# qmoututu11/Image_Restoration_and_Enhancement

Measured on AMD Instinct MI355X. Metric: restored images/sec @512x512, 50 DDIM steps; PSNR/SSIM vs reference, higher is better.
Workload: dtype bf16; 1 GPU; BASELINE configs[1] denoise 512x512, batch 8/GPU, 50 DDIM steps x strength 0.5 = 25 UNet evals, CFG 5.0 (UNet batch 16); task=denoise, global_batch=8, resolution=512, compute=UNet + CLIP bf16, VAE fp16 (fp32 accumulation), parallelism=dp1, weights_bcast=none, outputs_finite=True

## Files before the change

image_restoration_and_enhancement_amd/csrc/gemm_plan.cpp:

```cpp
#include "gemm_plan.h"

#include <algorithm>
#include <cmath>

namespace irx {

bool g_large_tiles = true;
int g_large_mask = 3;
int g_large_dense = 63;
int g_small_splitk = 1;
int g_gemm_sk = 1;
int g_gemm_deep = 0;
bool g_gemm_small = false;
int g_gemm_small_kmax = 1280;
int g_gemm_force = 0;
bool g_tile_256x320 = true;
bool g_splitk_inkernel = true;
int g_gemm_nmajor = 1;
int g_gemm_group = 1;
int g_gemm_pp = 2;
int g_gemm_pp2 = 1;
int g_gemm_pp_chain = 1;
int g_conv1x1_dense = 1;
int g_conv_halo = 1;
int g_halo_split = 1;
int g_halo_pipe = 1;
int g_halo_strip = 1;
int g_halo_up2 = 1;
int g_halo_mi = 1;
int g_halo_group = 1;
int g_gn_fuse = 0;
int g_gn_parts = 1;
int g_gn_red_parts = 1;
int g_gn_fold = 1;
int g_ln_fold = 1;
int g_ln_parts = 1;

namespace {

constexpr int kCUs = 256;
constexpr long kPairMinTiles = 2L * kCUs;

struct Choice {
  int BM = 0, BN = 0, splits = 1, per = 0;
  bool small = false;
  bool pair = false;
};

int step_k() { return g_gemm_deep == 1 ? 32 : 64; }

long canon_rows(const GemmArgs& a) {
  const long rows = (long)a.M * a.batch;
  return a.imgs > 0 ? rows / a.imgs * kCanonImages : rows;
}
int canon_batch(const GemmArgs& a) { return (a.imgs > 0 && a.batch > 1) ? kCanonImages : a.batch; }

bool reduce_in_kernel(int splits, long tiles) { return g_splitk_inkernel && splits == 2 && tiles <= kSplitCounters; }

Choice choose(const GemmArgs& a) {
  Choice best;
  const int nk = std::max(1, a.K / step_k());
  if (g_gemm_small && g_gemm_deep == 0 && a.K <= g_gemm_small_kmax) {
    const int bn = (!a.geglu && a.N % 160 == 0) ? 160 : (a.N % 128 == 0 ? 128 : 0);
    if (bn) {
      best.BM = 128; best.BN = bn; best.small = true; best.splits = 1; best.per = nk;
      return best;
    }
  }
  if (g_gemm_force > 0 && g_gemm_deep == 0) {
    const int BM = g_gemm_force / 100000, BN = (g_gemm_force / 100) % 1000, sp = g_gemm_force % 100;
    const bool ok = (BM == 256 || BM == 128 || (BM == 64 && BN == 320 && sp == 1 && !a.gn_part)) &&
                    (BN == 320 || BN == 256 || BN == 128) && a.N % BN == 0 &&
                    sp >= 1 && (sp == 1 || !((a.out_f32 && canon_batch(a) > 1) || a.geglu)) && (!a.geglu || BN % 128 == 0);
    if (ok) {
      best.BM = BM; best.BN = BN; best.splits = sp; best.per = (nk + sp - 1) / sp;
      if ((long)(sp - 1) * best.per < nk) return best;
    }
    best = Choice();
  }
  double best_score = -1.0;
  const int cands[7][2] = {{256, 320}, {256, 256}, {128, 320}, {256, 128}, {128, 256}, {128, 128}, {256, 160}};
  for (auto& c : cands) {
    const int BM = c[0], BN = c[1];
    if (BN == 160 && g_gemm_deep != 2) continue;
    if (BN == 320 && BM == 256 && (g_gemm_deep != 0 || !g_tile_256x320)) continue;
    if (a.N % BN != 0) continue;
    if (a.geglu && BN % 128 != 0) continue;
    const long tiles = (canon_rows(a) + BM - 1) / BM * (a.N / BN);
    const double eff = BM == 256 ? (BN >= 256 ? 1.0 : BN == 160 ? 0.9 : 0.65)
                                 : (BN == 320 ? 0.97 : BN == 256 ? 0.75 : 0.78);
    const int resident = (BM == 128 && BN == 128 && g_gemm_deep == 0) ? 2 : 1;
    const long cap = (long)kCUs * resident;
    for (int splits = 1; splits <= 8; splits *= 2) {
      if (splits > 1 && ((a.out_f32 && canon_batch(a) > 1) || a.geglu)) break;
      const int per = (nk + splits - 1) / splits;
      if (per * step_k() < 512 && splits > 1) break;
      if ((long)(splits - 1) * per >= nk) break;
      const long blocks = tiles * splits;
      const double util = (double)blocks / ((double)((blocks + cap - 1) / cap) * cap);
      const double cost_split = splits > 1 ? (1.0 + 0.35 * std::log2((double)splits)) * (per < 16 ? 1.6 : 1.0) : 1.0;
      const double score = util * eff / cost_split;
      if (score > best_score + 1e-9) {
        best_score = score;
        best.BM = BM; best.BN = BN; best.splits = splits; best.per = per;
      }
    }
  }
  return best;
}

bool vec_ok(const GemmArgs& a) {
  return !a.out_f32 && a.N % 8 == 0 && a.ldc % 8 == 0 && ((uintptr_t)a.C % 16) == 0 &&
         (!a.residual || (a.ldr % 8 == 0 && ((uintptr_t)a.residual % 16) == 0)) &&
         (a.batch == 1 || (a.sC % 8 == 0 && (!a.residual || a.sR % 8 == 0)));
}

bool pair_form(const GemmArgs& a) {
  return g_gemm_pp2 && g_gemm_pp && g_gemm_deep == 0 && !g_gemm_small && g_gemm_force == 0 && !a.conv && !a.A1 &&
         !a.b_rows && !a.rowadd && !a.gn_part && !a.gn_ab && !a.ln_out && !a.up2_w && a.K % 32 == 0;
}

bool pair_tile(const GemmArgs& a, const Choice& c, int& BM, int& BN) {
  if (!pair_form(a)) return false;
  int bm = 256, bn = 128;
  if (g_gemm_pp2 >= 2) {
    if (g_gemm_pp2 == 3) { bm = 128; bn = 256; }
  } else {
    if (c.splits != 1 || a.K % 64 != 0) return false;
    const long tiles = canon_rows(a) / bm * (a.N / bn);
    const bool geglu = a.geglu && c.BM == 256 && c.BN == 256 && tiles >= kCUs;
    const bool wide = !a.geglu && c.BM == 128 && c.BN == 320 && a.K >= 640 && tiles >= kPairMinTiles;
    if (!geglu && !wide) return false;
  }
  if (a.M % bm != 0 || a.N % bn != 0) return false;
  BM = bm; BN = bn;
  return true;
}

bool eligible(const GemmArgs& a) {
  const int bk = (g_gemm_pp2 >= 2 && pair_form(a)) ? 32 : step_k();
  if (!(g_large_mask & (a.conv ? 2 : 1))) return false;
  if (!a.conv && g_large_dense != 63) {
    const int cls = a.geglu ? (a.K <= 320 ? 4 : a.K <= 640 ? 16 : 32) : a.hs_L ? 2 : a.N <= 1280 ? 1 : 8;
    if (!(g_large_dense & cls)) return false;
  }
  if (a.hs_L && !vec_ok(a)) return false;
  if (a.act != ACT_NONE) return false;
  if (!vec_ok(a) && (a.rowadd || a.residual)) return false;
  if (a.rowadd && (a.rowadd_ld % 4 != 0 || ((uintptr_t)a.rowadd % 16) != 0)) return false;
  if (!is16(a.dtype) || a.K % bk != 0 || a.ldb % 8 != 0) return false;
  if (canon_rows(a) < 512) return false;
  if (a.geglu && (a.out_f32 || a.residual || a.batch != 1 || a.N % 128 != 0)) return false;
  if (a.conv) return !a.out_f32 && a.g.C0 % bk == 0 && a.g.C1 % bk == 0;
  if (a.A1 && (a.batch != 1 || a.kA1 % 64 != 0 || a.lda1 % 8 != 0 || ((uintptr_t)a.A1 % 16) != 0)) return false;
  return a.lda % 8 == 0 && (a.batch == 1 || a.sA % 8 == 0);
}

int small_splits(const GemmArgs& a) {
  if (!g_small_splitk || !is16(a.dtype) || a.conv || a.batch != 1 || a.geglu || a.A1 || a.up2_w) return 0;
  if (a.M > 256 || a.N % 8 || a.K < 1024 || a.N <= 16) return 0;
  if (a.out_f32 ? a.ldc % 4 != 0 : (a.ldc % 8 != 0 || ((uintptr_t)a.C % 16) != 0)) return 0;
  if (a.residual && (a.ldr % 8 != 0 || ((uintptr_t)a.residual % 16) != 0)) return 0;
  const long ctiles = (a.N + 63) / 64;
  if (ctiles >= 128) return 0;
  int sp = 1;
  while (sp < 8 && ctiles * sp * 2 <= 256 && a.K % (sp * 2 * 64) == 0 && a.K / (sp * 2) >= 256) sp *= 2;
  return sp > 1 ? sp : 0;
}

struct Halo {
  int mode = 0;
  int bn = 0;
  int splits = 1;
};

Halo plan_halo(const GemmArgs& a) {
  const ConvGeom& g = a.g;
  Halo h;
  if (!g_conv_halo || !a.conv || a.batch != 1 || a.geglu || a.out_f32 || !vec_ok(a)) return h;
  if (g.stride != 1) return h;
  if (a.up2_w) {
    if (!g_halo_up2 || !g_halo_pipe || a.gn_ab || g.KH != 2 || g.KW != 2 || (g.pad_t & ~1) || (g.pad_l & ~1)) return h;
  } else if (g.KH != 3 || g.KW != 3 || g.pad_t != 1 || g.pad_l != 1) {
    return h;
  }
  if (g.Hv != g.Hin || g.Wv != g.Win || g.Ho != g.Hin || g.Wo != g.Win) return h;
  if (g.C0 % 64 || g.C1 % 64 || g.C0 <= 0) return h;
  const int W = g.Win;
  if ((long)g.N * g.Hin * W != a.M) return h;
  const int slabs = (g.C0 + g.C1) / 64;
  const int bn = a.N % 160 == 0 ? 160 : (a.N % 128 == 0 && g_halo_pipe && !a.gn_ab) ? 128 : 0;
  if (W == 8 && g.Hin == 8 && g_halo_mi && g_halo_pipe && !a.gn_ab && a.M % 64 == 0) {
    if (bn != 160) return h;
    const long tiles = (canon_rows(a) + 255) / 256 * (a.N / bn);
    const int want = (int)std::max(1L, std::min(8L, (long)kCUs / std::max(1L, tiles)));
    const int per = (slabs + want - 1) / want;
    h.mode = 3; h.bn = bn; h.splits = (slabs + per - 1) / per;
    return h;
  }
  if (a.up2_w && ((long)a.up2_h * a.up2_w) % 256) return h;
  if (a.M % 256) return h;
  const bool rows = W >= 16 && W <= kHaloWMax && !(W & (W - 1)) && 256 % W == 0 && g.Hin % (256 / W) == 0;
  const bool strips = g_halo_strip && g_halo_pipe && !a.gn_ab && W % kStripW == 0 && g.Hin % (256 / kStripW) == 0;
  const int mode = strips && (g_halo_strip == 2 || !rows) ? 2 : rows ? 1 : 0;
  if (!mode || !bn) return h;
  const long tiles = canon_rows(a) / 256 * (a.N / bn);
  int splits = 0;
  if (tiles >= kCUs || g_conv_halo >= 2) splits = 1;
  else if (g_halo_split && 2 * tiles >= kCUs && slabs >= 8 && reduce_in_kernel(2, tiles)) splits = 2;
  if (!splits) return h;
  if (a.up2_w && mode == 2 && bn != 128) return h;
  static_assert((256 + 2 * kHaloWMax) * 8 <= 512 * 6, "halo normalisation chunks");
  h.mode = mode; h.bn = bn; h.splits = splits;
  return h;
}

int halo_group_m(const GemmArgs& a, const Halo& h) {
  if (!g_halo_group) return 0;
  const long tiles_m = (a.M + 255) / 256, tiles_n = a.N / h.bn;
  if (tiles_n < 2) return 0;
  const long q = (tiles_m * tiles_n + 7) / 8, w = std::min(q, 32L);
  const double hpix = h.mode == 2 ? 10.0 * (kStripW + 2) : 256.0 + 2.0 * a.g.Wo;
  const double a_m = hpix * (a.g.C0 + a.g.C1) * 2.0, b_n = (double)h.bn * a.K * 2.0;
  auto cost = [&](long g) {
    const bool whole = w >= g * tiles_n;
    const long gm = whole ? (w + tiles_n - 1) / tiles_n : std::min(g, w);
    const long gn = whole ? tiles_n : (w + g - 1) / g;
    return gm * a_m + gn * b_n;
  };
  const double legacy = cost(std::max(1L, (w + tiles_n - 1) / tiles_n));
  long best_g = 0;
  double best = legacy;
  for (long g = 1; g <= tiles_m; g *= 2)
    if (cost(g) < best) { best = cost(g); best_g = g; }
  return best < 0.9 * legacy ? (int)best_g : 0;
}

int dense_group_m(const GemmArgs& a, int bm, int bn, int resident, bool nmajor) {
  if (!g_gemm_group) return 0;
  const long tiles_m = (a.M + bm - 1) / bm, tiles_n = (a.N + bn - 1) / bn;
  if (tiles_n < 2 || tiles_m < 2) return 0;
  if (g_gemm_group >= 2) return (int)std::min((long)g_gemm_group, tiles_m);
  const long q = (tiles_m * tiles_n + 7) / 8, w = std::min(q, 32L * resident);
  const double a_m = (double)bm * a.K * 2.0, b_n = (double)bn * a.K * 2.0;
  auto cost = [&](long g) {
    const bool whole = w >= g * tiles_n;
    const long gm = whole ? (w + tiles_n - 1) / tiles_n : std::min(g, w);
    const long gn = whole ? tiles_n : (w + g - 1) / g;
    return gm * a_m + gn * b_n;
  };
  const double legacy = nmajor ? std::min(w, tiles_m) * a_m + (double)((w + tiles_m - 1) / tiles_m) * b_n
                               : cost(std::max(1L, (w + tiles_n - 1) / tiles_n));
  long best_g = 0;
  double best = legacy;
  for (long g = 1; g <= tiles_m; g *= 2)
    if (cost(g) < best) { best = cost(g); best_g = g; }
  return best < 0.9 * legacy ? (int)best_g : 0;
}

void set_kernel(GemmPlan& p, int BM, int BN, int WM, int WN, int BK, int S, int HALO = 0, bool PP = false) {
  p.BM = BM; p.BN = BN; p.WM = WM; p.WN = WN; p.BK = BK; p.S = S; p.HALO = HALO; p.PP = PP;
}

void plan_halo_launch(const GemmArgs& a, const Halo& h, GemmPlan& p) {
  p.path = GEMM_HALO;
  p.vec_epilogue = true;
  p.group_m = halo_group_m(a, h);
  const bool mi = h.mode == 3;
  int halo;
  if (mi) halo = a.up2_w ? 9 : 8;
  else if (a.up2_w) halo = h.mode == 2 ? 7 : 6;
  else if (h.mode == 2) halo = 5;
  else halo = g_halo_pipe && !a.gn_ab ? 2 : 1;
  set_kernel(p, 256, h.bn, 4, 2, 64, 3, halo);
  p.splits = h.splits;
  p.per = a.K / 64;
  if (h.splits > 1) {
    const int slabs = (a.g.C0 + a.g.C1) / 64;
    p.per = (a.up2_w ? 4 : 9) * ((slabs + h.splits - 1) / h.splits);
    p.Mp = (a.M + 255) / 256 * 256;
    p.Np = a.N;
    p.ws_bytes = (size_t)h.splits * p.Mp * a.N * sizeof(float);
    p.inkernel = !mi;
  }
}

bool large_kernel(const GemmArgs& a, const Choice& c, GemmPlan& p) {
  const int key = c.BM * 1000 + c.BN;
  const int wm = (c.BM == 256 && c.BN <= 160) ? 4 : 2, wn = 8 / wm;
  if (c.pair) {
    set_kernel(p, c.BM, c.BN, wm, wn, 32, 3, 0, true);
  } else if (c.BM == 64) {
    set_kernel(p, 64, 320, 1, 4, 32, 2);
  } else if (c.small) {
    set_kernel(p, 128, c.BN, 2, 2, 64, 2);
  } else if (g_gemm_deep == 0 && g_gemm_pp && !a.conv && !a.ln_out && !a.b_rows &&
             (!a.A1 || g_gemm_pp_chain) &&
             ((c.BM == 256 && c.BN == 256) ||
              (a.A1 && g_gemm_pp_chain && c.BN == 320 && (c.BM == 256 || c.BM == 128) && a.K >= 1024)) &&
             a.M % c.BM == 0 && a.N % c.BN == 0) {
    set_kernel(p, c.BM, c.BN, wm, wn, 32, 3, 0, true);
  } else if (g_gemm_deep == 2) {
    if (key == 256320) return false;
    set_kernel(p, c.BM, c.BN, wm, wn, 64, (key == 256256 || key == 128320) ? 2 : key == 128128 ? 4 : 3);
  } else if (g_gemm_deep == 1) {
    if (key == 256320 || c.BN == 160) return false;
    set_kernel(p, c.BM, c.BN, wm, wn, 32, key == 256256 ? 4 : key == 128128 ? 6 : 5);
  } else {
    if (c.BN == 160) return false;
    set_kernel(p, c.BM, c.BN, wm, wn, 64, 2);
  }
  return true;
}

bool plan_large(const GemmArgs& a, const Choice& c0, GemmPlan& p) {
  Choice c = c0;
  if (pair_tile(a, c0, c.BM, c.BN)) {
    c.pair = true;
    c.splits = 1;
  } else if (a.K % step_k() != 0) {
    return false;
  }
  const bool vec = vec_ok(a);
  if (a.geglu && !vec) return false;
  if (c.splits > 1) {
    if (!vec && !a.out_f32) return false;
    if (a.out_f32 && (a.ldc % 8 != 0 || a.N % 8 != 0)) return false;
  }
  if (!large_kernel(a, c, p)) return false;
  p.path = GEMM_LARGE;
  p.vec_epilogue = vec;
  p.nmajor = g_gemm_nmajor == 2 || (g_gemm_nmajor == 1 && (long)a.N * a.batch > (long)a.M * a.batch);
  if (a.batch == 1 && !a.hs_L) {
    p.group_m = dense_group_m(a, c.BM, c.BN, (c.BM == 128 && c.BN == 128) || c.small || c.pair ? 2 : 1, p.nmajor);
    if (p.group_m) p.nmajor = 0;
  }
  p.splits = c.splits;
  p.per = c.pair ? a.K / p.BK : (c.splits > 1 ? c.per : a.K / step_k()) * (step_k() / p.BK);
  if (c.splits > 1) {
    p.Mp = (a.M + c.BM - 1) / c.BM * c.BM;
    p.Np = (a.N + c.BN - 1) / c.BN * c.BN;
    p.ws_bytes = (size_t)c.splits * a.batch * p.Mp * p.Np * sizeof(float);
    p.inkernel = reduce_in_kernel(c.splits, (long)(p.Mp / c.BM) * (p.Np / c.BN) * a.batch);
  }
  return true;
}

template <typename T> T* requested() { return (T*)(uintptr_t)4096; }

}

bool gemm_sk_eligible(const GemmArgs& a) {
  if (!g_gemm_sk || (!a.geglu && g_gemm_sk != 3) || !is16(a.dtype) || a.conv || a.out_f32 || a.batch != 1 || a.K != kSkK) return false;
  if (a.act != ACT_NONE || a.rowadd || a.gn_part || a.gn_ab || a.b_rows || a.ln_out) return false;
  if (a.A1 || a.up2_w) return false;
  if (a.res_rows) return false;
  if (a.geglu ? (a.N % 256 != 0 || a.N / 2 / 128 > 32 || a.residual || a.hs_L || a.ldc % 4) : (a.N % 320 || a.N / 320 > 32))
    return false;
  if (a.lda % 8 || a.ldb % 8 || ((uintptr_t)a.A % 16) || ((uintptr_t)a.B % 16)) return false;
  if (((uintptr_t)a.C % 8) || (a.hs_L ? (a.hs_d % 4 || a.hs_C % 4) : a.ldc % 4)) return false;
  if (a.residual && (a.ldr % 4 || ((uintptr_t)a.residual % 8))) return false;
  if (a.hs_L && (a.residual || a.hs_L % 64)) return false;
  if ((a.ln_rs || a.ln_part) && (a.alpha != 1.f || a.M % 2)) return false;
  if (a.ln_part && a.ln_T != 1) return false;
  return a.M > 0;
}

GemmPlan gemm_plan(const GemmArgs& a) {
  GemmPlan p;
  const int small = small_splits(a);
  const size_t small_bytes = small ? (size_t)small * a.M * a.N * sizeof(float) : 0;
  p.ws_reserve = small_bytes;
  Halo h;
  Choice c;
  if (g_large_tiles && eligible(a)) {
    h = plan_halo(a);
    if (h.bn) {
      p.ws_reserve = h.splits > 1 ? (size_t)h.splits * ((a.M + 255) / 256 * 256) * a.N * sizeof(float) : 0;
    } else {
      c = choose(a);
      if (c.BM && c.splits > 1)
        p.ws_reserve = std::max(small_bytes, (size_t)c.splits * a.batch * ((a.M + c.BM - 1) / c.BM * c.BM) *
                                                 ((a.N + c.BN - 1) / c.BN * c.BN) * sizeof(float));
    }
    if (gemm_sk_eligible(a)) p.path = GEMM_SK;
    else if (h.bn) plan_halo_launch(a, h, p);
    else if (c.BM) plan_large(a, c, p);
  }
  if (p.path == GEMM_WAVE4 && small) {
    p.path = GEMM_WAVE4_SPLIT;
    p.splits = small;
    p.Mp = a.M; p.Np = a.N;
    p.ws_bytes = small_bytes;
  }

  const bool vec = p.vec_epilogue;
  const bool full_epi = p.large() && vec && (p.splits == 1 || p.inkernel);
  const bool one16 = a.batch == 1 && !a.out_f32;
  if (a.geglu) p.geglu = p.path == GEMM_SK ? vec_ok(a) : p.path == GEMM_LARGE && vec;
  if (a.up2_w) p.up2 = p.large() && vec && a.batch == 1 && !a.hs_L;
  if (a.gn_ab) p.gn_fused = g_gn_fuse && p.path == GEMM_HALO && p.HALO == 1;
  if (a.gn_part && g_gn_parts && p.large() && vec && one16 && !a.geglu && !a.hs_L) {
    if (p.splits > 1 && !p.inkernel)
      p.gn_rows = (g_gn_red_parts && !a.up2_w && !a.b_rows && a.M % kRedGnRows == 0 && a.N % 64 == 0 && a.act == ACT_NONE)
                      ? kRedGnRows : 0;
    else if (p.path == GEMM_HALO)
      p.gn_rows = h.mode == 3 ? 0 : 256;
    else if (a.up2_w && ((long)a.up2_h * a.up2_w) % p.BM)
      p.gn_rows = 0;
    else
      p.gn_rows = a.M % p.BM ? 0 : p.BM;
  }
  if (a.ln_rs || a.ln_part)
    p.ln_fold = !a.conv && a.alpha == 1.f && one16 && vec_ok(a) && (p.path == GEMM_SK || (p.path == GEMM_LARGE && full_epi));
  const bool staged = p.path == GEMM_LARGE && full_epi && !a.conv && one16 && !a.geglu && g_gemm_deep == 0;
  const bool ln_w_ok = a.ln_W == kLnGroup || a.ln_W == kLnGroupNarrow;
  if (a.ln_out && g_ln_parts && staged && !a.hs_L && !a.gn_part && ln_w_ok && a.N % a.ln_W == 0 &&
      !(a.ln_out_rs && a.N != a.ln_W)) {
    GemmArgs bare = a;
    bare.ln_out = nullptr;
    const bool tile = a.ln_W == kLnGroup ? (p.BM == 256 || p.BM == 128)
                                         : (p.BM == 128 && p.WM * p.WN == 8 && !p.PP);
    p.ln_out = p.BN == a.ln_W && tile && !gemm_sk_eligible(bare);
  }
  if (a.b_rows > 0)
    p.bimg = staged && !(p.WM == 2 && p.WN == 2) && a.M % a.b_rows == 0 && a.b_rows % p.BM == 0;
  return p;
}

size_t gemm_workspace_bytes(const GemmArgs& a) { return gemm_plan(a).ws_reserve; }

size_t gemm_small_split_bytes(const GemmArgs& a) {
  const int sp = small_splits(a);
  return sp ? (size_t)sp * a.M * a.N * sizeof(float) : 0;
}

int gemm_large_splits(const GemmArgs& a) {
  const GemmPlan p = gemm_plan(a);
  return p.large() ? p.splits : 0;
}

bool gemm_geglu_fusable(const GemmArgs& a) { return gemm_plan(a).geglu; }
bool gemm_up2_ok(const GemmArgs& a) { return gemm_plan(a).up2; }
bool gemm_bimg_ok(const GemmArgs& a) { return gemm_plan(a).bimg; }

int gemm_emits_gn_parts(const GemmArgs& a) {
  GemmArgs q = a;
  if (!q.gn_part) q.gn_part = requested<double>();
  return gemm_plan(q).gn_rows;
}

bool gemm_gn_fusable(const GemmArgs& a) {
  GemmArgs q = a;
  if (!q.gn_ab) q.gn_ab = requested<const float2>();
  return gemm_plan(q).gn_fused;
}

bool gemm_ln_foldable(const GemmArgs& a) {
  GemmArgs q = a;
  if (!q.ln_rs && !q.ln_part) q.ln_rs = requested<const float2>();
  return gemm_plan(q).ln_fold;
}

bool gemm_emits_ln_parts(const GemmArgs& a) {
  GemmArgs q = a;
  if (!q.ln_out) q.ln_out = requested<float2>();
  return gemm_plan(q).ln_out;
}

bool conv1x1_as_dense(GemmArgs& a) {
  const ConvGeom& g = a.g;
  if (!g_conv1x1_dense || !a.conv || !is16(a.dtype) || a.batch != 1 || a.gn_ab || a.up2_w || a.act != ACT_NONE) return false;
  if (g.KH != 1 || g.KW != 1 || g.stride != 1 || g.pad_t != 0 || g.pad_l != 0) return false;
  if (g.Hv != g.Hin || g.Wv != g.Win || g.Ho != g.Hin || g.Wo != g.Win) return false;
  GemmArgs d = a;
  d.conv = 0;
  d.g = ConvGeom();
  d.A = g.src0; d.lda = g.C0;
  d.A1 = g.C1 ? g.src1 : nullptr; d.lda1 = g.C1; d.kA1 = g.C1 ? g.C0 : 0;
  const int path = gemm_plan(d).path;
  if (path != GEMM_SK && path != GEMM_LARGE) return false;
  a = d;
  return true;
}

}
```

image_restoration_and_enhancement_amd/csrc/gemm_sk.hip:

```cpp
#include <algorithm>

#include "gemm_plan.h"
#include "profile.h"

#ifndef IRX_SK_DBG
#define IRX_SK_DBG 0
#endif

namespace irx {

int g_gemm_sk_blocks = 0;

namespace {

typedef __attribute__((address_space(3))) void lds_void;

__device__ __forceinline__ void glds16(const void* g, uint32_t lds_addr) {
  asm volatile("s_mov_b32 m0, %1\n\ts_nop 0\n\tglobal_load_lds_dwordx4 %0, off" ::"v"(g), "s"(lds_addr)
               : "memory", "m0");
}

__device__ __forceinline__ void vm_wait(int n) {
  switch (n) {
#define IRX_VM(k) case k: asm volatile("s_waitcnt vmcnt(" #k ")" ::: "memory"); break;
    IRX_VM(1) IRX_VM(2) IRX_VM(3) IRX_VM(4) IRX_VM(5) IRX_VM(6) IRX_VM(7) IRX_VM(8) IRX_VM(9) IRX_VM(10) IRX_VM(11)
    IRX_VM(12) IRX_VM(13) IRX_VM(14) IRX_VM(15) IRX_VM(16) IRX_VM(17) IRX_VM(18) IRX_VM(19) IRX_VM(20) IRX_VM(21)
    IRX_VM(22) IRX_VM(23) IRX_VM(24) IRX_VM(25) IRX_VM(26) IRX_VM(27) IRX_VM(28) IRX_VM(29) IRX_VM(30) IRX_VM(31)
    IRX_VM(32) IRX_VM(33) IRX_VM(34) IRX_VM(35) IRX_VM(36) IRX_VM(37) IRX_VM(38) IRX_VM(39) IRX_VM(40) IRX_VM(41)
    IRX_VM(42) IRX_VM(43) IRX_VM(44) IRX_VM(45) IRX_VM(46) IRX_VM(47) IRX_VM(48) IRX_VM(49) IRX_VM(50) IRX_VM(51)
    IRX_VM(52) IRX_VM(53) IRX_VM(54) IRX_VM(55) IRX_VM(56) IRX_VM(57) IRX_VM(58) IRX_VM(59) IRX_VM(60) IRX_VM(61)
    IRX_VM(62) IRX_VM(63)
#undef IRX_VM
    default: asm volatile("s_waitcnt vmcnt(0)" ::: "memory"); break;
  }
}

template <typename T> struct Pk;
template <> struct Pk<bf16_t> {
  __device__ static void unpack4(const uint2& u, float* f) {
    f[0] = __uint_as_float(u.x << 16); f[1] = __uint_as_float(u.x & 0xffff0000u);
    f[2] = __uint_as_float(u.y << 16); f[3] = __uint_as_float(u.y & 0xffff0000u);
  }
};
template <> struct Pk<f16_t> {
  __device__ static void unpack4(const uint2& u, float* f) {
    const f16x4 h = __builtin_bit_cast(f16x4, u);
    f[0] = (float)h[0]; f[1] = (float)h[1]; f[2] = (float)h[2]; f[3] = (float)h[3];
  }
};

constexpr int kSkKS = kSkK / 32;
constexpr int kSkRC = kSkK / 8;

template <typename T, int NB, bool GEGLU, int MB, int BPC, bool RES, int S, bool AF2>
__global__ __launch_bounds__(256, BPC) void gemm_sk_kernel(GemmArgs a, int n_slices, int groups) {
  constexpr int BM = 16 * MB, KS = kSkKS, RC = kSkRC;
  constexpr int STAGE = BM * RC;
  constexpr int PPW = STAGE / 64 / 4;
  static_assert(PPW * 256 == STAGE, "whole pieces per wave");
  constexpr int NS = 4 * NB * 16;
  static_assert(!GEGLU || NB == 4, "GEGLU: 2 value + 2 gate blocks per wave");
  static_assert(!(RES && GEGLU), "no residual on the GEGLU projection");
  constexpr int OC = GEGLU ? 32 : NB * 16;
  constexpr int CH = OC / 8;
  constexpr int SRU = CH + 1;
  constexpr int NR = MB / 2;
  constexpr int NCK = 32 * CH / 64;
  static_assert(MB % 2 == 0 && (32 * CH) % 64 == 0, "32-row rounds, whole chunks per lane");
  constexpr int RESN = RES ? NR * NCK : 0;
  constexpr int LNL = BM / 8;
  constexpr int SN = NR * NCK;
  __shared__ __attribute__((aligned(16))) uint4 ring[S * STAGE];
  __shared__ __attribute__((aligned(16))) float2 lnring[S * BM];
  __shared__ __attribute__((aligned(16))) uint4 resbuf[RES ? 2 * 4 * BM * CH : 1];
  __shared__ __attribute__((aligned(16))) float sbias[NS];
  __shared__ __attribute__((aligned(16))) float su[NS];
  __shared__ __attribute__((aligned(16))) uint4 stage_buf[4 * 32 * SRU];
  __shared__ long noff_tab[4 * CH];

  const int tid = threadIdx.x, lane = tid & 63;
  const int w = __builtin_amdgcn_readfirstlane(tid >> 6);
  auto spare = [](int r, int rem) { return r < rem ? r : (rem > 1 ? (r & 1) : 0); };
  const int x = blockIdx.x & 7, loc = blockIdx.x >> 3;
  const int sl = loc % n_slices, grp = loc / n_slices;
  if (grp >= groups) return;
  const int tiles = (a.M + BM - 1) / BM;
  const int lo = (int)((long)x * tiles / 8), hi = (int)((long)(x + 1) * tiles / 8);
  const int t0 = lo + grp;
  if (t0 >= hi) return;
  const int nt = (hi - t0 + groups - 1) / groups;
  const bool has_ln = !RES && (a.ln_rs != nullptr || a.ln_part != nullptr);
  const float2* const lnsrc = a.ln_part ? a.ln_part : a.ln_rs;
  const int PA = PPW + (has_ln ? 1 : 0);

  auto wrow = [&](int idx) -> int {
    if constexpr (!GEGLU) {
      return sl * NS + idx;
    } else {
      const int wv = idx / (NB * 16), j = (idx / 16) % NB, q = idx & 15;
      const int o = sl * 128 + wv * 32 + (j & 1) * 16 + q;
      return (o >> 6) * 128 + (j >= 2 ? 64 : 0) + (o & 63);
    }
  };
  for (int i = tid; i < NS; i += 256) {
    const int n = wrow(i);
    sbias[i] = a.bias ? a.bias[n] : 0.f;
    su[i] = a.ln_u ? a.ln_u[n] : 0.f;
  }
  const int n0w = GEGLU ? sl * 128 + w * 32 : sl * NS + w * OC;
  long* const ncol = noff_tab + w * CH;
  if (lane < CH) {
    const int n = n0w + lane * 8;
    long o = n;
    if (a.hs_L) {
      const int part = n / a.hs_C, rm = n - part * a.hs_C, hd = rm / a.hs_d, e = rm - hd * a.hs_d;
      o = (long)part * a.M * a.hs_C + (long)hd * a.hs_L * a.hs_d + e;
    }
    ncol[lane] = o;
  }

  uint4 bfr[NB][KS];
#pragma unroll
  for (int j = 0; j < NB; ++j) {
    const int n = wrow((w * NB + j) * 16 + (lane & 15));
    const uint16_t* p = (const uint16_t*)a.B + (long)n * a.ldb + (lane >> 4) * 8;
#pragma unroll
    for (int kk = 0; kk < KS; ++kk) bfr[j][kk] = *(const uint4*)(p + kk * 32);
  }
  __builtin_amdgcn_s_waitcnt(0x0F70);

  auto tile_of = [&](int it) { return t0 + min(it, nt - 1) * groups; };
  auto lds32 = [](const void* p) { return __builtin_amdgcn_readfirstlane((uint32_t)(uintptr_t)(lds_void*)p); };
  const uint16_t* Ag = (const uint16_t*)a.A;
  auto issueA = [&](int it) {
    const long m0 = (long)tile_of(it) * BM;
    const int rem = a.M - (int)m0;
    const uint16_t* base = Ag + m0 * a.lda;
    uint4* st = ring + (it % S) * STAGE + w * PPW * 64;
#pragma unroll
    for (int j = 0; j < PPW; ++j) {
      const int p = (w * PPW + j) * 64 + lane;
      const int r = p / RC, c = (p % RC) ^ (r & 7);
      glds16(base + spare(r, rem) * a.lda + c * 8, lds32(st + j * 64));
    }
    if (has_ln) {
      if (lane < LNL) {
        const int r = 2 * (w * LNL + lane);
        glds16(lnsrc + m0 + (r < rem ? r : 0), lds32(lnring + (it % S) * BM + 2 * w * LNL));
      }
    }
  };
  auto issueR = [&](int it) {
    if constexpr (RES) {
      const long m0 = (long)tile_of(it) * BM;
      const int rem = a.M - (int)m0;
      const uint16_t* R = (const uint16_t*)a.residual + m0 * a.ldr + n0w;
      uint4* dst = resbuf + ((it & 1) * 4 + w) * BM * CH;
#pragma unroll
      for (int k = 0; k < RESN; ++k) {
        const int p = lane + 64 * k, r = p / CH, c = p % CH;
        glds16(R + spare(r, rem) * a.ldr + c * 8, lds32(dst + 64 * k));
      }
    }
  };

  uint4* const stg = stage_buf + w * 32 * SRU;
  const int q4 = (lane >> 4) * 4;
  auto crow = [&](int k) { return (lane + 64 * k) / CH; };
  auto cch = [&](int k) { return (lane + 64 * k) % CH; };
  const long rstride = a.hs_L ? a.hs_d : a.ldc;

  const int sw = lane & 7, hb = sw >> 2, lo4 = (lane >> 4) ^ (sw & 3);
  const int fb0 = (lane & 15) * RC + 4 * hb + lo4, fb1 = (lane & 15) * RC + 4 * (hb ^ 1) + lo4;

#pragma unroll
  for (int p = 0; p < S - 1; ++p)
    if constexpr (!(IRX_SK_DBG & 4)) issueA(p);
  issueR(0);
  for (int it = 0; it < nt; ++it) {
    if constexpr (!(IRX_SK_DBG & 4))
      vm_wait(min(63, it <= S - 2 ? (S - 2 - it) * PA + RESN + it * (RESN + PA + SN)
                                  : SN + (S - 2) * (RESN + PA + SN)));
    asm volatile("s_waitcnt lgkmcnt(0)\n\ts_barrier" ::: "memory");
    issueR(it + 1);
    if constexpr (!(IRX_SK_DBG & 4)) issueA(it + S - 1);
    const uint4* As = ring + (it % S) * STAGE;
    f32x4 acc[NB][MB];
#pragma unroll
    for (int j = 0; j < NB; ++j)
#pragma unroll
      for (int i = 0; i < MB; ++i) acc[j][i] = f32x4{0.f, 0.f, 0.f, 0.f};
    if constexpr (!(IRX_SK_DBG & 2)) {
      constexpr int NAF = AF2 ? 2 : 1;
      uint4 af[NAF][MB];
      auto rdA = [&](int kk, uint4* f) {
        const int fb = (kk & 1) ? fb1 : fb0;
#pragma unroll
        for (int i = 0; i < MB; ++i) f[i] = As[fb + 8 * (kk >> 1) + i * 16 * RC];
      };
      if constexpr (AF2) rdA(0, af[0]);
#pragma unroll
      for (int kk = 0; kk < KS; ++kk) {
        if constexpr (AF2) {
          if (kk + 1 < KS) rdA(kk + 1, af[(kk + 1) & 1]);
        } else {
          rdA(kk, af[0]);
        }
        __builtin_amdgcn_s_setprio(1);
#pragma unroll
        for (int j = 0; j < NB; ++j)
#pragma unroll
          for (int i = 0; i < MB; ++i) acc[j][i] = Mfma<T>::m16x16x32(bfr[j][kk], af[AF2 ? (kk & 1) : 0][i], acc[j][i]);
        __builtin_amdgcn_s_setprio(0);
      }
    }
    if constexpr ((IRX_SK_DBG & 1) != 0) {
      float t = 0.f;
#pragma unroll
      for (int j = 0; j < NB; ++j)
#pragma unroll
        for (int i = 0; i < MB; ++i) t += acc[j][i][0] + acc[j][i][3];
      if (t == 12345.678f) ((float*)a.C)[lane] = t;
      continue;
    }

    if constexpr (RES) vm_wait(min(63, it == 0 ? RESN + PA : 2 * PA + SN + RESN));
    const long tm0 = (long)tile_of(it) * BM;
    const int rem = a.M - (int)tm0;
    long mbase = tm0 * a.ldc;
    if (a.hs_L) {
      const long img = tm0 / a.hs_L;
      mbase = img * a.hs_C * a.hs_L + (tm0 - img * a.hs_L) * a.hs_d;
    }
    const float2* lst = lnring + (it % S) * BM;
    const uint4* rsb = resbuf + ((it & 1) * 4 + w) * BM * CH;
    T* Cp = (T*)a.C;
#pragma unroll
    for (int rr = 0; rr < NR; ++rr) {
#pragma unroll
      for (int ih = 0; ih < 2; ++ih) {
        const int i = 2 * rr + ih;
        float2 rs = has_ln ? lst[i * 16 + (lane & 15)] : make_float2(1.f, 0.f);
        if (a.ln_part) rs = ln_fin(rs.x, rs.y, 1, a.ln_eps);
        float v[NB][4];
#pragma unroll
        for (int j = 0; j < NB; ++j) {
          const float4 bb = *(const float4*)(sbias + (w * NB + j) * 16 + q4);
          const float bj[4] = {bb.x, bb.y, bb.z, bb.w};
          if (has_ln) {
            const float4 uu = *(const float4*)(su + (w * NB + j) * 16 + q4);
            const float uj[4] = {uu.x, uu.y, uu.z, uu.w};
#pragma unroll
            for (int r = 0; r < 4; ++r) v[j][r] = Mfma<T>::round(fmaf(acc[j][i][r], rs.x, fmaf(-rs.y, uj[r], bj[r])));
          } else {
#pragma unroll
            for (int r = 0; r < 4; ++r) v[j][r] = Mfma<T>::round(acc[j][i][r] * a.alpha + bj[r]);
          }
        }
        uint2* srow = (uint2*)(stg + (ih * 16 + (lane & 15)) * SRU) + (lane >> 4);
        if constexpr (GEGLU) {
#pragma unroll
          for (int jj = 0; jj < 2; ++jj) {
            float o[4];
#pragma unroll
            for (int r = 0; r < 4; ++r) o[r] = v[jj][r] * gelu_erf16(v[jj + 2][r]);
            srow[jj * 4] = make_uint2(Mfma<T>::pack2(o[0], o[1]), Mfma<T>::pack2(o[2], o[3]));
          }
        } else {
#pragma unroll
          for (int j = 0; j < NB; ++j)
            srow[j * 4] = make_uint2(Mfma<T>::pack2(v[j][0], v[j][1]), Mfma<T>::pack2(v[j][2], v[j][3]));
        }
      }
#pragma unroll
      for (int k = 0; k < NCK; ++k) {
        uint4 u = stg[crow(k) * SRU + cch(k)];
        if constexpr (!GEGLU) {
          if (RES || a.out_scale != 1.f) {
            float f[8];
            Vec16<T>::unpack(u, f);
            if constexpr (RES) {
              float rv[8];
              Vec16<T>::unpack(rsb[rr * 32 * CH + lane + 64 * k], rv);
#pragma unroll
              for (int e = 0; e < 8; ++e) f[e] += rv[e];
            }
#pragma unroll
            for (int e = 0; e < 8; ++e) f[e] *= a.out_scale;
            u = Vec16<T>::pack(f);
          }
        }
        const int row = rr * 32 + crow(k);
        const int srow2 = spare(row, rem);
        *(uint4*)(Cp + mbase + srow2 * rstride + ncol[cch(k)]) = u;
      }
    }
  }
  asm volatile("s_waitcnt vmcnt(0)" ::: "memory");
}

template <typename T, int NB, bool GEGLU, int MB, int BPC, bool RES, int S, bool AF2>
void launch_sk(const GemmArgs& a, hipStream_t s) {
  constexpr int NS = 4 * NB * 16;
  const int n_slices = GEGLU ? (a.N / 2) / 128 : a.N / NS;
  const int per_xcd = std::max(n_slices, g_gemm_sk_blocks > 0 ? g_gemm_sk_blocks : 32 * BPC);
  const int groups = per_xcd / n_slices;
  const char* tn = std::is_same<T, f16_t>::value ? "_Float16" : "unsigned short";
  std::string nm;
  if (prof_on())
    nm = std::string("irx::(anonymous namespace)::gemm_sk_kernel<") + tn + ", " + std::to_string(NB) + ", " +
         (GEGLU ? "true" : "false") + ", " + std::to_string(MB) + ", " + std::to_string(BPC) + ", " +
         (RES ? "true" : "false") + ", " + std::to_string(S) + ", " + (AF2 ? "true" : "false") + ">";
  if (prof_on() && g_prof_shapes)
    nm += " [M " + std::to_string(a.M) + " N " + std::to_string(a.N) + " K " + std::to_string(a.K) + "]";
  ProfScope ps(nm, 2.0 * a.M * a.N * (double)a.K, s);
  gemm_sk_kernel<T, NB, GEGLU, MB, BPC, RES, S, AF2><<<8 * per_xcd, 256, 0, s>>>(a, n_slices, groups);
  IRX_LAUNCH_CHECK();
}

}

bool gemm_sk(const GemmArgs& a0, hipStream_t s) {
  if (!gemm_sk_eligible(a0)) return false;
  const GemmArgs& a = a0;
  const bool f16 = a.dtype == F16;
  if (a.geglu) {
    if (g_gemm_sk == 2) {
      if (f16) launch_sk<f16_t, 4, true, 4, 1, false, 3, true>(a, s);
      else launch_sk<bf16_t, 4, true, 4, 1, false, 3, true>(a, s);
    } else {
      if (f16) launch_sk<f16_t, 4, true, 2, 2, false, 3, false>(a, s);
      else launch_sk<bf16_t, 4, true, 2, 2, false, 3, false>(a, s);
    }
  } else if (a.residual) {
    if (f16) launch_sk<f16_t, 5, false, 2, 1, true, 4, true>(a, s);
    else launch_sk<bf16_t, 5, false, 2, 1, true, 4, true>(a, s);
  } else {
    if (f16) launch_sk<f16_t, 5, false, 4, 1, false, 3, true>(a, s);
    else launch_sk<bf16_t, 5, false, 4, 1, false, 3, true>(a, s);
  }
  return true;
}

}
```

Baseline: 19.03 images/s.

## Software-pipeline GEGLU split-K GEMM epilogue into next tile's MFMA loop

Adds a PIPE variant of the persistent split-K GEMM kernel for the GEGLU projection, and makes it the default by setting g_gemm_sk to 4. The GELU gating, LDS staging and global stores for tile it-1 are interleaved across the K-step MFMA loop of tile it using sched_group_barrier and setprio, with a drain epilogue after the loop. The aim is to hide the epilogue's VALU and store latency behind matrix-core work instead of running it serially after each tile. In exchange the kernel keeps packed results in registers across iterations, which adds register pressure and depends on fragile instruction-scheduling hints.

```diff
diff --git a/image_restoration_and_enhancement_amd/csrc/gemm_plan.cpp b/image_restoration_and_enhancement_amd/csrc/gemm_plan.cpp
--- a/image_restoration_and_enhancement_amd/csrc/gemm_plan.cpp
+++ b/image_restoration_and_enhancement_amd/csrc/gemm_plan.cpp
@@ -9,7 +9,7 @@
 int g_large_mask = 3;
 int g_large_dense = 63;
 int g_small_splitk = 1;
-int g_gemm_sk = 1;
+int g_gemm_sk = 4;
 int g_gemm_deep = 0;
 bool g_gemm_small = false;
 int g_gemm_small_kmax = 1280;
diff --git a/image_restoration_and_enhancement_amd/csrc/gemm_sk.hip b/image_restoration_and_enhancement_amd/csrc/gemm_sk.hip
--- a/image_restoration_and_enhancement_amd/csrc/gemm_sk.hip
+++ b/image_restoration_and_enhancement_amd/csrc/gemm_sk.hip
@@ -37,12 +37,19 @@
 
 template <typename T> struct Pk;
 template <> struct Pk<bf16_t> {
+  __device__ static void unpack2(uint32_t u, float* f) {
+    f[0] = __uint_as_float(u << 16); f[1] = __uint_as_float(u & 0xffff0000u);
+  }
   __device__ static void unpack4(const uint2& u, float* f) {
     f[0] = __uint_as_float(u.x << 16); f[1] = __uint_as_float(u.x & 0xffff0000u);
     f[2] = __uint_as_float(u.y << 16); f[3] = __uint_as_float(u.y & 0xffff0000u);
   }
 };
 template <> struct Pk<f16_t> {
+  __device__ static void unpack2(uint32_t u, float* f) {
+    const f16x2 h = __builtin_bit_cast(f16x2, u);
+    f[0] = (float)h[0]; f[1] = (float)h[1];
+  }
   __device__ static void unpack4(const uint2& u, float* f) {
     const f16x4 h = __builtin_bit_cast(f16x4, u);
     f[0] = (float)h[0]; f[1] = (float)h[1]; f[2] = (float)h[2]; f[3] = (float)h[3];
@@ -52,7 +59,7 @@
 constexpr int kSkKS = kSkK / 32;
 constexpr int kSkRC = kSkK / 8;
 
-template <typename T, int NB, bool GEGLU, int MB, int BPC, bool RES, int S, bool AF2>
+template <typename T, int NB, bool GEGLU, int MB, int BPC, bool RES, int S, bool AF2, int PIPE>
 __global__ __launch_bounds__(256, BPC) void gemm_sk_kernel(GemmArgs a, int n_slices, int groups) {
   constexpr int BM = 16 * MB, KS = kSkKS, RC = kSkRC;
   constexpr int STAGE = BM * RC;
@@ -137,9 +144,11 @@
     const int rem = a.M - (int)m0;
     const uint16_t* base = Ag + m0 * a.lda;
     uint4* st = ring + (it % S) * STAGE + w * PPW * 64;
+    int ln = lane;
+    if constexpr (PIPE != 0) asm volatile("" : "+v"(ln));
 #pragma unroll
     for (int j = 0; j < PPW; ++j) {
-      const int p = (w * PPW + j) * 64 + lane;
+      const int p = (w * PPW + j) * 64 + ln;
       const int r = p / RC, c = (p % RC) ^ (r & 7);
       glds16(base + spare(r, rem) * a.lda + c * 8, lds32(st + j * 64));
     }
@@ -172,6 +181,133 @@
 
   const int sw = lane & 7, hb = sw >> 2, lo4 = (lane >> 4) ^ (sw & 3);
   const int fb0 = (lane & 15) * RC + 4 * hb + lo4, fb1 = (lane & 15) * RC + 4 * (hb ^ 1) + lo4;
+
+  if constexpr (PIPE != 0) {
+    static_assert(GEGLU && MB == 2 && NCK == 2 && !RES, "the pipelined loop: the two-per-CU GEGLU form");
+    uint32_t cv[MB][NB][2];
+    T* const Cp = (T*)a.C;
+    auto fold = [&](const f32x4 (&acc)[NB][MB], int it) {
+      const float2* lst = lnring + (it % S) * BM;
+#pragma unroll
+      for (int i = 0; i < MB; ++i) {
+        float2 rs = has_ln ? lst[i * 16 + (lane & 15)] : make_float2(1.f, 0.f);
+        if (a.ln_part) rs = ln_fin(rs.x, rs.y, 1, a.ln_eps);
+#pragma unroll
+        for (int j = 0; j < NB; ++j) {
+          const float4 bb = *(const float4*)(sbias + (w * NB + j) * 16 + q4);
+          const float bj[4] = {bb.x, bb.y, bb.z, bb.w};
+          float v[4];
+          if (has_ln) {
+            const float4 uu = *(const float4*)(su + (w * NB + j) * 16 + q4);
+            const float uj[4] = {uu.x, uu.y, uu.z, uu.w};
+#pragma unroll
+            for (int r = 0; r < 4; ++r) v[r] = fmaf(acc[j][i][r], rs.x, fmaf(-rs.y, uj[r], bj[r]));
+          } else {
+#pragma unroll
+            for (int r = 0; r < 4; ++r) v[r] = acc[j][i][r] * a.alpha + bj[r];
+          }
+          cv[i][j][0] = Mfma<T>::pack2(v[0], v[1]);
+          cv[i][j][1] = Mfma<T>::pack2(v[2], v[3]);
+        }
+        __builtin_amdgcn_sched_barrier(0);
+      }
+    };
+    auto gelu2 = [&](int g, int half) -> uint32_t {
+      float h[2], gg[2];
+      Pk<T>::unpack2(cv[g >> 1][g & 1][half], h);
+      Pk<T>::unpack2(cv[g >> 1][(g & 1) + 2][half], gg);
+      return Mfma<T>::pack2(h[0] * gelu_erf16(gg[0]), h[1] * gelu_erf16(gg[1]));
+    };
+    auto stage_wr = [&](int g, uint32_t lo, uint32_t hi) {
+      uint2* srow = (uint2*)(stg + ((g >> 1) * 16 + (lane & 15)) * SRU) + (lane >> 4);
+      srow[(g & 1) * 4] = make_uint2(lo, hi);
+    };
+    auto out_ptr = [&](int pit, int k) -> uint4* {
+      const long tm0 = (long)tile_of(pit) * BM;
+      return (uint4*)(Cp + tm0 * a.ldc + spare(crow(k), a.M - (int)tm0) * rstride + ncol[cch(k)]);
+    };
+    auto mma_tile = [&](int it, auto epi) {
+      constexpr bool EPI = decltype(epi)::value;
+      const uint4* As = ring + (it % S) * STAGE;
+      f32x4 acc[NB][MB];
+#pragma unroll
+      for (int j = 0; j < NB; ++j)
+#pragma unroll
+        for (int i = 0; i < MB; ++i) acc[j][i] = f32x4{0.f, 0.f, 0.f, 0.f};
+      uint4 af[1][MB];
+      uint32_t o01 = 0;
+      uint4 u0, u1;
+      auto rdA1 = [&](int kk, int i) {
+        return As[((kk & 1) ? fb1 : fb0) + 8 * (kk >> 1) + i * 16 * RC];
+      };
+      af[0][0] = rdA1(0, 0);
+      af[0][1] = rdA1(0, 1);
+      __builtin_amdgcn_sched_barrier(0);
+#pragma unroll
+      for (int kk = 0; kk < KS; ++kk) {
+        __builtin_amdgcn_s_setprio(1);
+#pragma unroll
+        for (int i = 0; i < MB; ++i) {
+#pragma unroll
+          for (int j = 0; j < NB; ++j) acc[j][i] = Mfma<T>::m16x16x32(bfr[j][kk], af[0][i], acc[j][i]);
+          if (kk + 1 < KS) af[0][i] = rdA1(kk + 1, i);
+        }
+        if constexpr (EPI) {
+          if (kk < 8) {
+            const uint32_t pk = gelu2(kk >> 1, kk & 1);
+            if (kk & 1) stage_wr(kk >> 1, o01, pk);
+            else o01 = pk;
+          } else if (kk == 8) {
+            u0 = stg[crow(0) * SRU + cch(0)];
+            u1 = stg[crow(1) * SRU + cch(1)];
+          } else {
+            *out_ptr(it - 1, 0) = u0;
+            *out_ptr(it - 1, 1) = u1;
+          }
+        }
+#pragma unroll
+        for (int m = 0; m < NB * MB; ++m) {
+          __builtin_amdgcn_sched_group_barrier(0x008, 1, 0);
+          if constexpr (EPI) {
+            if (m & 1) __builtin_amdgcn_sched_group_barrier(0x402, 4, 0);
+            else __builtin_amdgcn_sched_group_barrier(0x402, 5, 0);
+            if (m == 3) {
+              if (kk < 8) __builtin_amdgcn_sched_group_barrier(0x200, 1, 0);
+              else if (kk == 8) __builtin_amdgcn_sched_group_barrier(0x100, NCK + 2, 0);
+              else __builtin_amdgcn_sched_group_barrier(0x040, NCK, 0);
+            }
+          }
+          if ((m == 3 || m == 7) && kk + 1 < KS) __builtin_amdgcn_sched_group_barrier(0x100, 1, 0);
+        }
+        __builtin_amdgcn_s_setprio(0);
+        __builtin_amdgcn_sched_barrier(0);
+      }
+      fold(acc, it);
+    };
+#pragma unroll
+    for (int p = 0; p < S - 1; ++p) issueA(p);
+    for (int it = 0; it < nt; ++it) {
+      vm_wait((S - 2) * PA + min(max(it - 1, 0), S - 1) * SN);
+      asm volatile("s_waitcnt lgkmcnt(0)\n\ts_barrier" ::: "memory");
+      issueA(it + S - 1);
+      __builtin_amdgcn_sched_barrier(0);
+      if (it > 0) mma_tile(it, std::true_type());
+      else mma_tile(it, std::false_type());
+    }
+    {
+      uint32_t o01 = 0;
+#pragma unroll
+      for (int g2 = 0; g2 < 8; ++g2) {
+        const uint32_t pk = gelu2(g2 >> 1, g2 & 1);
+        if (g2 & 1) stage_wr(g2 >> 1, o01, pk);
+        else o01 = pk;
+      }
+#pragma unroll
+      for (int k = 0; k < NCK; ++k) *out_ptr(nt - 1, k) = stg[crow(k) * SRU + cch(k)];
+    }
+    asm volatile("s_waitcnt vmcnt(0)" ::: "memory");
+    return;
+  }
 
 #pragma unroll
   for (int p = 0; p < S - 1; ++p)
@@ -299,7 +435,7 @@
   asm volatile("s_waitcnt vmcnt(0)" ::: "memory");
 }
 
-template <typename T, int NB, bool GEGLU, int MB, int BPC, bool RES, int S, bool AF2>
+template <typename T, int NB, bool GEGLU, int MB, int BPC, bool RES, int S, bool AF2, int PIPE = 0>
 void launch_sk(const GemmArgs& a, hipStream_t s) {
   constexpr int NS = 4 * NB * 16;
   const int n_slices = GEGLU ? (a.N / 2) / 128 : a.N / NS;
@@ -310,11 +446,12 @@
   if (prof_on())
     nm = std::string("irx::(anonymous namespace)::gemm_sk_kernel<") + tn + ", " + std::to_string(NB) + ", " +
          (GEGLU ? "true" : "false") + ", " + std::to_string(MB) + ", " + std::to_string(BPC) + ", " +
-         (RES ? "true" : "false") + ", " + std::to_string(S) + ", " + (AF2 ? "true" : "false") + ">";
+         (RES ? "true" : "false") + ", " + std::to_string(S) + ", " + (AF2 ? "true" : "false") + ", " +
+         std::to_string(PIPE) + ">";
   if (prof_on() && g_prof_shapes)
     nm += " [M " + std::to_string(a.M) + " N " + std::to_string(a.N) + " K " + std::to_string(a.K) + "]";
   ProfScope ps(nm, 2.0 * a.M * a.N * (double)a.K, s);
-  gemm_sk_kernel<T, NB, GEGLU, MB, BPC, RES, S, AF2><<<8 * per_xcd, 256, 0, s>>>(a, n_slices, groups);
+  gemm_sk_kernel<T, NB, GEGLU, MB, BPC, RES, S, AF2, PIPE><<<8 * per_xcd, 256, 0, s>>>(a, n_slices, groups);
   IRX_LAUNCH_CHECK();
 }
 
@@ -325,6 +462,13 @@
   const GemmArgs& a = a0;
   const bool f16 = a.dtype == F16;
   if (a.geglu) {
+#if IRX_SK_DBG == 0
+    if (g_gemm_sk == 4) {
+      if (f16) launch_sk<f16_t, 4, true, 2, 2, false, 3, false, 1>(a, s);
+      else launch_sk<bf16_t, 4, true, 2, 2, false, 3, false, 1>(a, s);
+      return true;
+    }
+#endif
     if (g_gemm_sk == 2) {
       if (f16) launch_sk<f16_t, 4, true, 4, 1, false, 3, true>(a, s);
       else launch_sk<bf16_t, 4, true, 4, 1, false, 3, true>(a, s);
```

Result: no change. 18.99 images/s (-0.2%).
